# HakimNessah/th_rl

Hardware: NVIDIA B200
Metric: agent-steps/sec (higher is better)
Workload: dtype f32

## Files before the change

th_rl_b200/csrc/thrl.cu:

```cuda
#include <cuda_runtime.h>
#include <stdarg.h>
#include <stdio.h>
#include <string.h>

#include <math.h>
#include <stdlib.h>

#include <algorithm>
#include <array>
#include <cmath>
#include <atomic>
#include <map>
#include <memory>
#include <mutex>
#include <set>
#include <vector>

#include "thrl_device.cuh"
#include "thrl_scan_generic.cuh"
#include "thrl_scan_hbm.cuh"
#include "thrl_scan_lut2.cuh"
#include "thrl_scan_lpc.cuh"
#include "thrl_scan_mixed.cuh"
#include "thrl_scan_pwl.cuh"
// ... 463 lines not shown
    }
    state_of[j] = it->second;
  }
  const int NS = (int)tuples.size();
  if (NS > thrl::kLut2MaxStates) return false;
  std::set<int> rows[2];
  for (auto& t : tuples) { rows[0].insert(t[0]); rows[0].insert(t[1]); rows[1].insert(t[2]); rows[1].insert(t[3]); }
  if (noisy) {
    if (NS + 1 + T > 255) return false;
    for (int a = 0; a < 2; ++a) {
      if (!rows[a].empty() && *rows[a].rbegin() > rmax[a]) return false;
      for (int r = 0; r <= rmax[a]; ++r) rows[a].insert(r);
    }
  }
  std::map<int, int> cidx[2];
  for (int a = 0; a < 2; ++a) {
    if ((int)rows[a].size() > thrl::kLut2MaxRows) return false;
    int c = 0;
    for (int row : rows[a]) {
      if (row < 0 || row > G.agent[a].states) return false;
      p->row_list[a][c] = (uint16_t)row;
      cidx[a][row] = c++;
    }
    p->NR[a] = c;
    const ThrlAgentSpec& s = G.agent[a];
    p->L[a] = s.min_memory > s.capacity ? 0 : (T < s.capacity ? T : s.capacity);
  }
  p->J = J;
  p->NS = NS;
  for (int j = 0; j < J; ++j) p->next_state[j] = (uint8_t)state_of[j];
  for (int s = 0; s < NS; ++s) {
    const auto& t = tuples[s];
    p->state_rows[s] = (uint32_t)cidx[0][t[0]] | ((uint32_t)cidx[0][t[1]] << 8) | ((uint32_t)cidx[1][t[2]] << 16) |
                       ((uint32_t)cidx[1][t[3]] << 24);
  }
  int o = 0;
  p->off_next = o;    o += align_up(2 * J, 16);
  p->off_rowlist = o; o += align_up(2 * (p->NR[0] + p->NR[1]), 16);
  p->off_lutlog = o;  o += J * 32;
  p->off_lutr = o;
  p->cta_bytes_lpc = o + J * 16;
  o += align_up(J * 8, 16);
  p->off_aq = o;      o += align_up((A0 + A1) * 8, 16);
  p->cta_bytes = o;
  o = align_up((p->NR[0] + 2) * A0 * (int)elem, 16);
  p->off_tab1 = o;    o += align_up((p->NR[1] + 2) * A1 * (int)elem, 16);
  p->off_grow = o;    o += align_up(p->NR[0] + p->NR[1] + 4, 16);
  const int nstates = NS + 1 + (noisy ? T : 0);
  p->off_rows = o;    o += align_up(nstates * 4, 16);
  {
    const int gj = align_up((NS + 2) * 4, 16), scr = thrl::kLut2Chunk * 8 + 16;
    p->off_gj = o;    o += gj > scr ? gj : scr;
    p->off_scr = p->off_gj;
  }
  p->off_nt = o;      o += noisy ? align_up(T, 16) : 0;
  p->off_nrec = o;    o += noisy ? align_up(T * 8, 16) : 0;
  p->off_seq = o;     o += noisy ? align_up(T + 1, 16) : 0;
  p->off_rec = o;     o += align_up(2 * T, 16);
  {
    const int pre = align_up(T * 8, 16), olds = align_up(2 * T * (int)elem, 16);
    p->off_old = o;   o += pre > olds ? pre : olds;
  }
  p->warp_bytes = o;
  const int w = (smem_optin - p->cta_bytes) / p->warp_bytes;
  if (w < 2) return false;
  int wmax = elem == 8 ? thrl::Lut2Warps<double>::kMax : thrl::Lut2Warps<float>::kMax;
  if (noisy && wmax > thrl::kLut2NoiseWarps) wmax = thrl::kLut2NoiseWarps;
  *warps = w > wmax ? wmax : w;
  return true;
}

template <typename QT>
int launch_lut2(thrl::Lut2Params& p, int warps, const DeviceInfo& dev, cudaStream_t stream) {
  int grid = dev.sms;
  g_last_wave = (long long)dev.sms * warps;
  const long long needed_ctas = (p.n_runs + warps - 1) / warps;
  if (needed_ctas < grid) {
    warps = (int)((p.n_runs + dev.sms - 1) / dev.sms);
    if (warps < 1) warps = 1;
    grid = (int)((p.n_runs + warps - 1) / warps);
  }
  const size_t smem = (size_t)p.cta_bytes + (size_t)warps * p.warp_bytes;
  const bool small = p.game.agent[0].actions <= 32 && p.game.agent[1].actions <= 32;
  auto kern = p.noisy ? (small ? thrl::qtable_scan_lut2<QT, true, true> : thrl::qtable_scan_lut2<QT, false, true>)
                      : (small ? thrl::qtable_scan_lut2<QT, true> : thrl::qtable_scan_lut2<QT, false>);
  CUDA_TRY(cudaFuncSetAttribute(kern, cudaFuncAttributeMaxDynamicSharedMemorySize, (int)smem));
  g_last_kernel = "lut2";
  kern<<<grid, warps * 32, smem, stream>>>(p);
  CUDA_TRY(cudaGetLastError());
  g_launches.fetch_add(1);
  return THRL_OK;
}

template <typename QT, int GL>
int launch_lpc_gl(thrl::Lut2Params& p, const DeviceInfo& dev, cudaStream_t stream) {
  const ThrlGame& G = p.game;
  const int T = G.max_steps, esz = (int)sizeof(QT);
  thrl::LpcLayout lay;
  lay.cells_max = 0; lay.rows_max = 0;
  int Lmax = 1;
  for (int a = 0; a < 2; ++a) {
    const int cells = (p.NR[a] + 2) * G.agent[a].actions;
    if (cells > lay.cells_max) lay.cells_max = cells;
    if (p.NR[a] + 2 > lay.rows_max) lay.rows_max = p.NR[a] + 2;
    if (p.L[a] > Lmax) Lmax = p.L[a];
  }
  int o = 0;
  lay.off_tab = o;  o += align_up(lay.cells_max * GL * esz, 16);
  lay.off_old = o;  o += align_up(Lmax * GL * esz, 16);
  lay.off_rec = o;  o += align_up(T * GL * 4, 16);
  lay.off_pre = o;  o += align_up(T * GL, 16);
  lay.off_gj = o;   o += align_up((p.NS + 1) * GL * 4, 16);
  lay.off_rows = o; o += align_up((p.NS + 1) * GL * 2, 16);
  lay.off_grow = o; o += align_up(lay.rows_max * GL, 16);
  lay.off_eps = o;  o += align_up(GL * 8, 16);
  lay.off_xrow = o; o += align_up(2 * GL * 2, 16);
  lay.warp_bytes = o;
  int warps = (dev.smem_optin - p.cta_bytes_lpc) / lay.warp_bytes;
  if (warps < 1) return fail(THRL_ERR_UNSUPPORTED, "lpc: one warp group needs %d B of shared memory", lay.warp_bytes);
  if (warps > thrl::kLpcMaxWarps) warps = thrl::kLpcMaxWarps;
  const long long groups = (p.n_runs + GL / 2 - 1) / (GL / 2);
  int grid = dev.sms;
  if ((groups + warps - 1) / warps < grid) {
    warps = (int)((groups + dev.sms - 1) / dev.sms);
    if (warps < 1) warps = 1;
    grid = (int)((groups + warps - 1) / warps);
  }
  const size_t smem = (size_t)p.cta_bytes_lpc + (size_t)warps * lay.warp_bytes;
  const bool a21 = G.agent[0].actions == 21 && G.agent[1].actions == 21;
  auto kern = a21 ? thrl::qtable_scan_lpc<QT, GL, 21> : thrl::qtable_scan_lpc<QT, GL, 0>;
  CUDA_TRY(cudaFuncSetAttribute(kern, cudaFuncAttributeMaxDynamicSharedMemorySize, (int)smem));
  g_last_kernel = "lpc";
  g_last_wave = (long long)grid * warps * (GL / 2);
  kern<<<grid, warps * 32, smem, stream>>>(p, lay);
  CUDA_TRY(cudaGetLastError());
  g_launches.fetch_add(1);
  return THRL_OK;
}
template <typename QT>
int launch_lpc(thrl::Lut2Params& p, const DeviceInfo& dev, cudaStream_t stream) {
  const char* s = getenv("THRL_LPC_GL");
  const int gl = s ? atoi(s) : 8;
  switch (gl) {
    case 4: return launch_lpc_gl<QT, 4>(p, dev, stream);
    case 16: return launch_lpc_gl<QT, 16>(p, dev, stream);
    default: return launch_lpc_gl<QT, 8>(p, dev, stream);
  }
}

template <typename QT>
int launch_mixed(thrl::MixedParams& p, const DeviceInfo& dev, cudaStream_t stream) {
  const ThrlGame& G = p.game;
  const int n = G.n_agents, T = G.max_steps, Hp = p.Hp, esz = (int)sizeof(QT);
  int lut = 0, par = 0, pmax = 0, hmax = 0, amax = 0;
  for (int i = 0; i < n; ++i) {
    const ThrlAgentSpec& s = G.agent[i];
    lut += s.actions;
    p.par_off[i] = 0;
    if (s.kind == THRL_AGENT_QTABLE) continue;
    const int P = s.kind == THRL_AGENT_CAC ? 5 * s.hidden + 3 : 2 * s.hidden + s.actions * s.hidden + s.actions + (s.kind == THRL_AGENT_ACTORCRITIC ? s.hidden + 1 : 0);
    p.par_off[i] = par;
    par += align_up(P, 4);
    if (P > pmax) pmax = P;
    if (s.hidden > hmax) hmax = s.hidden;
    if (s.actions > amax) amax = s.actions;
  }
  p.lut_total = lut;
  p.cta_bytes = align_up(2 * lut * 8, 16);
  int o = 0;
  p.off_P = o;    o += align_up(Hp * 8, 16);
// ... 897 lines not shown
```

th_rl_b200/csrc/thrl_scan_lut2.cuh:

```cuda
#pragma once
#include "thrl_device.cuh"

namespace thrl {

constexpr int kLut2MaxJoint = 1024;
constexpr int kLut2MaxStates = 254;
constexpr int kLut2MaxRows = 253;

struct Lut2Params {
  ThrlGame game;
  long long n_runs, run_id0;
  int epoch_begin, E, rng_mode;
  uint32_t k0, k1;
  void* q;
  uint32_t* counter;
  double* eps;
  double* price;
  const double* hp;
  const double* replay_u;
  const int32_t* replay_ra;
  double* rewards_log;
  double* actions_log;
  long long n_log_runs;
  long long* stats;
  int32_t* trace_actions;
  double* trace_rewards;
  double* trace_prices;
  int J, NS, NR[2], L[2];
  uint8_t next_state[kLut2MaxJoint];
  uint32_t state_rows[kLut2MaxStates];
  uint16_t row_list[2][kLut2MaxRows + 3];
  int cta_bytes, warp_bytes;
  int cta_bytes_lpc;
  int off_next, off_rowlist, off_lutlog, off_lutr, off_aq;
  int off_tab1, off_grow, off_rows, off_gj, off_seq, off_rec, off_scr, off_old;
  int noisy;
  int off_nt, off_nrec;
  const double* replay_new_a;
};

constexpr int kLut2MaxWarps = 24;
template <typename QT> struct Lut2Warps { static constexpr int kMax = kLut2MaxWarps; };
template <> struct Lut2Warps<double> { static constexpr int kMax = 16; };
constexpr int kLut2NoiseWarps = 16;
constexpr int kLut2Chunk = 16;

template <typename QT, bool kSmallA>
__device__ __forceinline__ QT lut2_row_max(const QT* row_lane, int A, int lane, bool in) {
  QT m = in ? row_lane[0] : NegInf<QT>::v();
  if (!kSmallA) {
    for (int k = lane + 32; k < A; k += 32) { const QT v = row_lane[k - lane]; m = v > m ? v : m; }
  }
  return warp_max(m);
}
template <typename QT, bool kSmallA>
__device__ __forceinline__ int lut2_row_argmax(const QT* row, int A, int lane, bool in) {
  if (!kSmallA) return row_argmax(row, A, lane);
  const QT v = in ? row[lane] : NegInf<QT>::v();
  const QT wm = warp_max(v);
  return (int)__reduce_min_sync(kFull, (in && v == wm) ? (unsigned)lane : 0xffffffffu);
}

template <typename QT, bool kSmallA, bool kNoise = false>
__global__ void __launch_bounds__(kNoise ? 32 * kLut2NoiseWarps : 32 * Lut2Warps<QT>::kMax, 1) qtable_scan_lut2(const __grid_constant__ Lut2Params p) {
  extern __shared__ __align__(16) unsigned char smem[];
  const ThrlGame& G = p.game;
  const int lane = threadIdx.x & 31, warps_per_cta = blockDim.x >> 5;
  const int warp = __shfl_sync(kFull, (int)(threadIdx.x >> 5), 0);
  const int T = G.max_steps, E = p.E, J = p.J, NS = p.NS;
  const int A0 = G.agent[0].actions, A1 = G.agent[1].actions;
  const int NR0 = p.NR[0], NR1 = p.NR[1];
  const int rng_mode = p.rng_mode;
  const uint32_t key0 = p.k0, key1 = p.k1;

  uint16_t* nextS = reinterpret_cast<uint16_t*>(smem + p.off_next);
  uint16_t* rowlist = reinterpret_cast<uint16_t*>(smem + p.off_rowlist);
  double* lutP = reinterpret_cast<double*>(smem + p.off_lutr);
  double* lutAq = reinterpret_cast<double*>(smem + p.off_aq);
  double* lutLog = reinterpret_cast<double*>(smem + p.off_lutlog);
  {
    const double ab = __ddiv_rn(G.a, G.b);
    for (int j = threadIdx.x; j < J; j += blockDim.x) {
      const int k0 = j / A1, k1 = j - k0 * A1;
      const double x0 = scale_action(k0, A0, G.agent[0].action_lo, G.agent[0].action_hi);
      const double x1 = scale_action(k1, A1, G.agent[1].action_lo, G.agent[1].action_hi);
      const double aq0 = __dmul_rn(ab, x0), aq1 = __dmul_rn(ab, x1);
      const double Q = __dadd_rn(__dadd_rn(0.0, aq0), aq1);
      const double pn = __dsub_rn(G.a, __dmul_rn(G.b, Q));
      const double price = pn > 0.0 ? pn : (pn != pn ? pn : 0.0);
      const double r0 = __dmul_rn(price, aq0), r1 = __dmul_rn(price, aq1);
      lutP[j] = price;
      lutLog[4 * j + 0] = __ddiv_rn(r0, (double)T);
      lutLog[4 * j + 1] = __ddiv_rn(r1, (double)T);
      lutLog[4 * j + 2] = __ddiv_rn(x0, (double)T);
      lutLog[4 * j + 3] = __ddiv_rn(x1, (double)T);
      nextS[j] = (uint16_t)(4u * p.next_state[j]);
    }
    for (int k = threadIdx.x; k < A0 + A1; k += blockDim.x) {
      const ThrlAgentSpec& sa = G.agent[k < A0 ? 0 : 1];
      lutAq[k] = __dmul_rn(ab, scale_action(k < A0 ? k : k - A0, sa.actions, sa.action_lo, sa.action_hi));
    }
    for (int c = threadIdx.x; c < NR0 + NR1; c += blockDim.x)
      rowlist[c] = c < NR0 ? p.row_list[0][c] : p.row_list[1][c - NR0];
  }
  __syncthreads();

  unsigned char* slot = smem + p.cta_bytes + (size_t)warp * p.warp_bytes;
  QT* tab0 = reinterpret_cast<QT*>(slot);
  QT* tab1 = reinterpret_cast<QT*>(slot + p.off_tab1);
  uint8_t* grow = slot + p.off_grow;
  uint32_t* rowsW = reinterpret_cast<uint32_t*>(slot + p.off_rows);
  unsigned char* GJb = slot + p.off_gj;
  uint32_t* GJ = reinterpret_cast<uint32_t*>(GJb);
  uint16_t* rec = reinterpret_cast<uint16_t*>(slot + p.off_rec);
  uint8_t* seq = slot + p.off_seq;
  uint2* pre = reinterpret_cast<uint2*>(slot + p.off_old);
  unsigned char* chunk = slot + p.off_scr;
  QT* olds = reinterpret_cast<QT*>(slot + p.off_old);
  uint8_t* nT = slot + p.off_nt;
  double* nrec = reinterpret_cast<double*>(slot + p.off_nrec);

  const bool in0 = lane < A0, in1 = lane < A1;
  const bool hi_half = lane >= 16;
  const int L0 = p.L[0], L1 = p.L[1];
  const uint32_t dp_b = (uint32_t)A1 | (1u << 8);
  const uint32_t tab0_off = (uint32_t)(reinterpret_cast<unsigned char*>(tab0) - smem);
  const uint32_t tab1_off = (uint32_t)(reinterpret_cast<unsigned char*>(tab1) - smem);
  const uint32_t tab0_lane_off = tab0_off + (uint32_t)sizeof(QT) * (uint32_t)(kSmallA ? (lane < A0 ? lane : A0 - 1) : lane);
// ... 78 lines not shown
    uint32_t sig4 = 4u * (uint32_t)NS;
    int last_k = -1;
    double noise_price = -1.0;

    for (int e = 0; e < E; ++e) {
      const uint32_t eabs = (uint32_t)(p.epoch_begin + e);
      const long long step0 = (r * E + e) * (long long)T;

      const unsigned long long thr0 = u32_unit_threshold(eps0), thr1 = u32_unit_threshold(eps1);
      for (int t = lane; t < T; t += 32) {
        int f0, f1;
        if (rng_mode == THRL_RNG_PHILOX) {
          uint32_t x[4];
          philox4x32_10(gid, eabs, (uint32_t)t, kStreamAct << 16, key0, key1, x);
          f0 = x[0] < thr0 ? (int)__umulhi(x[1], (uint32_t)A0) : -1;
          f1 = x[2] < thr1 ? (int)__umulhi(x[3], (uint32_t)A1) : -1;
        } else if (rng_mode == THRL_RNG_REPLAY_DRAWS) {
          const double2 u = *reinterpret_cast<const double2*>(p.replay_u + (step0 + t) * 2);
          const int2 v = *reinterpret_cast<const int2*>(p.replay_ra + (step0 + t) * 2);
          f0 = u.x < eps0 ? v.x : -1;
          f1 = u.y < eps1 ? v.y : -1;
        } else {
          const int2 v = *reinterpret_cast<const int2*>(p.replay_ra + (step0 + t) * 2);
          f0 = v.x; f1 = v.y;
        }
        pre[t] = make_uint2((f0 < 0 ? 0xffu : 0u) | (f1 < 0 ? 0xff00u : 0u),
                            (uint32_t)(f0 < 0 ? 0 : f0) | ((uint32_t)(f1 < 0 ? 0 : f1) << 8));
      }
      int nK = 0;
      if (kNoise) {
        for (int t0 = 0; t0 < T; t0 += 32) {
          const int t = t0 + lane;
          bool ev = false;
          double na = G.a;
          if (t < T) {
            if (rng_mode == THRL_RNG_PHILOX) {
              uint32_t x[4];
              philox4x32_10(gid, eabs, (uint32_t)t, kStreamEnv << 16, key0, key1, x);
              if (u53(x[0], x[1]) < G.noise_prob) {
                const double lo = __dmul_rn(G.a, 0.7);
                na = __dadd_rn(lo, __dmul_rn(__dsub_rn(G.a, lo), u53(x[2], x[3])));
                ev = true;
              }
            } else if (p.replay_new_a) {
              na = p.replay_new_a[step0 + t];
              ev = __double_as_longlong(na) != __double_as_longlong(G.a);
            }
          }
          const unsigned m = __ballot_sync(kFull, ev);
          if (ev) {
            const int idx = nK + __popc(m & ((1u << lane) - 1u));
            nT[idx] = (uint8_t)t;
            nrec[idx] = na;
          }
          nK += __popc(m);
        }
      }
      __syncwarp();

      const uint32_t sig4_start = sig4;
      double acc = 0.0;
      {
        const uint32_t base = (uint32_t)__cvta_generic_to_shared(smem);
        const uint32_t pre_a = base + (uint32_t)(reinterpret_cast<unsigned char*>(pre) - smem);
        const uint32_t rec_a = base + (uint32_t)(reinterpret_cast<unsigned char*>(rec) - smem);
        const uint32_t gj_a = base + (uint32_t)(GJb - smem);
        const uint32_t log_a = base + (uint32_t)p.off_lutlog + 8u * (uint32_t)(lane & 3);
        uint32_t next_a = base + (uint32_t)p.off_next;
        asm volatile("" : "+r"(next_a));
        const uint32_t log_lane = lane < 4 ? 1u : 0u;
        double lg = 0.0;
        uint32_t kk = 0;
        auto step = [&](uint32_t fx, uint32_t fy) {
          uint32_t gj, s16;
          asm volatile("ld.shared.u32 %0, [%1];" : "=r"(gj) : "r"(gj_a + sig4));
          kk = (gj & fx) | fy;
          const uint32_t joint = __dp4a(kk, dp_b, 0u);
          asm volatile("{ .reg .pred q; setp.ne.u32 q, %2, 0; @q ld.shared.f64 %0, [%1]; }"
                       : "+d"(lg) : "r"(log_a + 32u * joint), "r"(log_lane));
          acc = __dadd_rn(acc, lg);
          asm volatile("ld.shared.u16 %0, [%1];" : "=r"(s16) : "r"(next_a + 2u * joint));
          sig4 = s16;
        };
        if (!kNoise) {
        uint32_t pa = pre_a, ra = rec_a;
#pragma unroll 2
        for (int n2 = T >> 1; n2 > 0; --n2, pa += 16u, ra += 4u) {
          uint32_t f0x, f0y, f1x, f1y;
          asm volatile("ld.shared.v4.u32 {%0, %1, %2, %3}, [%4];" : "=r"(f0x), "=r"(f0y), "=r"(f1x), "=r"(f1y) : "r"(pa));
          step(f0x, f0y);
          const uint32_t ka = kk;
          step(f1x, f1y);
          asm volatile("st.shared.u32 [%0], %1;" ::"r"(ra), "r"(__byte_perm(ka, kk, 0x5410)) : "memory");
        }
        if (T & 1) {
          uint32_t fx, fy;
          asm volatile("ld.shared.v2.u32 {%0, %1}, [%2];" : "=r"(fx), "=r"(fy) : "r"(pa));
          step(fx, fy);
          asm volatile("st.shared.u16 [%0], %1;" ::"r"(ra), "h"((uint16_t)kk) : "memory");
        }
        } else {
          auto single = [&](int t) {
            uint32_t fx, fy;
            asm volatile("ld.shared.v2.u32 {%0, %1}, [%2];" : "=r"(fx), "=r"(fy) : "r"(pre_a + 8u * (uint32_t)t));
            step(fx, fy);
            asm volatile("st.shared.u16 [%0], %1;" ::"r"(rec_a + 2u * (uint32_t)t), "h"((uint16_t)kk) : "memory");
          };
          const double ab = __ddiv_rn(G.a, G.b), Td = (double)T;
          int t = 0;
          for (int k = 0; k <= nK; ++k) {
            const int tn = k < nK ? (int)nT[k] : T;
            if (t < tn && (t & 1)) { single(t); ++t; }
            for (; t + 1 < tn; t += 2) {
              uint32_t f0x, f0y, f1x, f1y;
              asm volatile("ld.shared.v4.u32 {%0, %1, %2, %3}, [%4];" : "=r"(f0x), "=r"(f0y), "=r"(f1x), "=r"(f1y) : "r"(pre_a + 8u * (uint32_t)t));
              step(f0x, f0y);
              const uint32_t ka = kk;
              step(f1x, f1y);
              asm volatile("st.shared.u32 [%0], %1;" ::"r"(rec_a + 2u * (uint32_t)t), "r"(__byte_perm(ka, kk, 0x5410)) : "memory");
            }
            if (t < tn) { single(t); ++t; }
            if (tn < T) {
              uint32_t fx, fy, gj;
              asm volatile("ld.shared.v2.u32 {%0, %1}, [%2];" : "=r"(fx), "=r"(fy) : "r"(pre_a + 8u * (uint32_t)tn));
              asm volatile("ld.shared.u32 %0, [%1];" : "=r"(gj) : "r"(gj_a + sig4));
              kk = (gj & fx) | fy;
              const int k0 = (int)(kk & 0xff), k1 = (int)(kk >> 8);
              const uint32_t joint = __dp4a(kk, dp_b, 0u);
              const double aq0 = __dmul_rn(ab, scale_action(k0, A0, G.agent[0].action_lo, G.agent[0].action_hi));
              const double aq1 = __dmul_rn(ab, scale_action(k1, A1, G.agent[1].action_lo, G.agent[1].action_hi));
              const double na = nrec[k];
              const double pn = __dsub_rn(na, __dmul_rn(G.b, __dadd_rn(__dadd_rn(0.0, aq0), aq1)));
              const double np = pn > 0.0 ? pn : (pn != pn ? pn : 0.0);
              const double r0 = __dmul_rn(np, aq0), r1 = __dmul_rn(np, aq1);
              if (lane < 2) lg = __ddiv_rn(lane == 0 ? r0 : r1, Td);
              else if (lane < 4) lg = lutLog[4 * joint + lane];
              acc = __dadd_rn(acc, lg);
              const int ta0 = act_row(np, (float)G.agent[0].max_state, (float)G.agent[0].states);
              const int tu0 = upd_row(np, G.agent[0].max_state, (double)G.agent[0].states);
              const int ta1 = act_row(np, (float)G.agent[1].max_state, (float)G.agent[1].states);
              const int tu1 = upd_row(np, G.agent[1].max_state, (double)G.agent[1].states);
              __syncwarp();
              if (lane == 0) {
                nrec[k] = np;
                rowsW[NS + 1 + k] = (uint32_t)ta0 | ((uint32_t)tu0 << 8) | ((uint32_t)ta1 << 16) | ((uint32_t)tu1 << 24);
                GJ[NS + 1] = (uint32_t)grow[ta0] | ((uint32_t)grow[NR0 + 2 + ta1] << 8);
                rec[tn] = (uint16_t)kk;
              }
              __syncwarp();
              sig4 = 4u * (uint32_t)(NS + 1);
              t = tn + 1;
            }
          }
        }
        last_k = (int)kk;
      }
      __syncwarp();
      if (kNoise) {
        for (int t = lane; t <= T; t += 32) {
          uint32_t s4 = sig4_start;
          if (t > 0) { const uint32_t kk = rec[t - 1]; s4 = nextS[__dp4a(kk, dp_b, 0u)]; }
          seq[t] = (uint8_t)(s4 >> 2);
        }
        __syncwarp();
        for (int k = lane; k < nK; k += 32) seq[nT[k] + 1] = (uint8_t)(NS + 1 + k);
        __syncwarp();
      }
// ... 145 lines not shown
            const QT v = row[k];
            if (v > m) { m = v; g = k; }
          }
          return g;
        };
        const unsigned w0a = __reduce_or_sync(kFull, dirty0a), w0b = __reduce_or_sync(kFull, dirty0b);
        const unsigned w1a = __reduce_or_sync(kFull, dirty1a), w1b = __reduce_or_sync(kFull, dirty1b);
        const unsigned below = (1u << lane) - 1u;
        const int n0a = __popc(w0a), n0 = n0a + __popc(w0b), n1a = n0 + __popc(w1a), nd = n1a + __popc(w1b);
        uint8_t* dlist = reinterpret_cast<uint8_t*>(olds);
        if ((w0a >> lane) & 1u) dlist[__popc(w0a & below)] = (uint8_t)lane;
        if ((w0b >> lane) & 1u) dlist[n0a + __popc(w0b & below)] = (uint8_t)(32 + lane);
        if ((w1a >> lane) & 1u) dlist[n0 + __popc(w1a & below)] = (uint8_t)lane;
        if ((w1b >> lane) & 1u) dlist[n1a + __popc(w1b & below)] = (uint8_t)(32 + lane);
        __syncwarp();
        for (int i = lane; i < nd; i += 32) {
          const bool ag = i >= n0;
          const int c = dlist[i], A = ag ? A1 : A0;
          grow[(ag ? NR0 + 2 : 0) + c] = (uint8_t)scan_row((ag ? tab1 : tab0) + c * A, A);
        }
        if (__any_sync(kFull, dirty_all0))
          for (int c = 64 + lane; c < NR0 + 2; c += 32) grow[c] = (uint8_t)scan_row(tab0 + c * A0, A0);
        if (__any_sync(kFull, dirty_all1))
          for (int c = 64 + lane; c < NR1 + 2; c += 32) grow[NR0 + 2 + c] = (uint8_t)scan_row(tab1 + c * A1, A1);
        __syncwarp();
        if (kNoise && sig4 > 4u * (uint32_t)NS) {
          if (lane == 0) rowsW[NS] = rowsW[NS + nK];
          noise_price = nrec[nK - 1];
          sig4 = 4u * (uint32_t)NS;
          __syncwarp();
        } else if (kNoise) {
          noise_price = -1.0;
        }
        for (int s = lane; s <= NS; s += 32) {
          const uint32_t rw = rowsW[s];
          GJ[s] = (uint32_t)grow[rw & 0xff] | ((uint32_t)grow[NR0 + 2 + ((rw >> 16) & 0xff)] << 8);
        }
      }
      {
        const double epsend0 = hparam(0, 2), epsstep0 = hparam(0, 3), epsend1 = hparam(1, 2), epsstep1 = hparam(1, 3);
        eps0 = __dadd_rn(epsend0, __dmul_rn(__dsub_rn(eps0, epsend0), epsstep0));
        eps1 = __dadd_rn(epsend1, __dmul_rn(__dsub_rn(eps1, epsend1), epsstep1));
      }
      if (lane < 4) {
        const int ag = lane & 1;
        if (r < p.n_log_runs) {
          double* dst = lane < 2 ? p.rewards_log : p.actions_log;
          if (dst) dst[(r * E + e) * 2 + ag] = acc;
        }
        if (p.stats) {
          unsigned long long* s4 = reinterpret_cast<unsigned long long*>(p.stats) + ((size_t)e * 2 + ag) * THRL_STATS_K + (lane < 2 ? 0 : 2);
          atomicAdd(s4 + 0, (unsigned long long)fx_round(__dmul_rn(acc, THRL_STATS_SCALE_SUM)));
          atomicAdd(s4 + 1, (unsigned long long)fx_round(__dmul_rn(__dmul_rn(acc, acc), THRL_STATS_SCALE_SQ)));
        }
      }
      __syncwarp();
    }

    for (int c = 0; c < NR0 + 2; ++c) {
      const int row = table_row0(c);
      if (row >= 0) for (int k = lane; k < A0; k += 32) qg0[(size_t)row * G.agent[0].row_stride + k] = tab0[c * A0 + k];
    }
    for (int c = 0; c < NR1 + 2; ++c) {
      const int row = table_row1(c);
      if (row >= 0) for (int k = lane; k < A1; k += 32) qg1[(size_t)row * G.agent[1].row_stride + k] = tab1[c * A1 + k];
    }
    if (lane == 0) {
      p.eps[r * 2] = eps0;
      p.eps[r * 2 + 1] = eps1;
      if (kNoise && noise_price >= 0.0) {
        p.price[r] = noise_price;
      } else if (last_k >= 0) {
        const double ab = __ddiv_rn(G.a, G.b);
        const double aq0 = __dmul_rn(ab, scale_action(last_k & 0xff, A0, G.agent[0].action_lo, G.agent[0].action_hi));
        const double aq1 = __dmul_rn(ab, scale_action(last_k >> 8, A1, G.agent[1].action_lo, G.agent[1].action_hi));
        const double pn = __dsub_rn(G.a, __dmul_rn(G.b, __dadd_rn(__dadd_rn(0.0, aq0), aq1)));
        p.price[r] = pn > 0.0 ? pn : (pn != pn ? pn : 0.0);
      }
    }
    __syncwarp();
  }
}

}
```

Before: 31.16 billion.

## Add paired-run LUT2 kernel processing two runs per warp with half-warp split

```diff
diff --git a/th_rl_b200/csrc/thrl.cu b/th_rl_b200/csrc/thrl.cu
--- a/th_rl_b200/csrc/thrl.cu
+++ b/th_rl_b200/csrc/thrl.cu
@@ -569,10 +569,21 @@
   }
   const size_t smem = (size_t)p.cta_bytes + (size_t)warps * p.warp_bytes;
   const bool small = p.game.agent[0].actions <= 32 && p.game.agent[1].actions <= 32;
+  g_last_kernel = "lut2";
   auto kern = p.noisy ? (small ? thrl::qtable_scan_lut2<QT, true, true> : thrl::qtable_scan_lut2<QT, false, true>)
-                      : (small ? thrl::qtable_scan_lut2<QT, true> : thrl::qtable_scan_lut2<QT, false>);
+                      : thrl::qtable_scan_lut2<QT, false>;
+  if constexpr (std::is_same<QT, float>::value) {
+    if (small && !p.noisy) {
+      CUDA_TRY(cudaFuncSetAttribute(thrl::qtable_scan_lut2_pair, cudaFuncAttributeMaxDynamicSharedMemorySize, (int)smem));
+      thrl::qtable_scan_lut2_pair<<<grid, (warps + 1) / 2 * 32, smem, stream>>>(p, warps);
+      CUDA_TRY(cudaGetLastError());
+      g_launches.fetch_add(1);
+      return THRL_OK;
+    }
+  } else if (small && !p.noisy) {
+    kern = thrl::qtable_scan_lut2<QT, true>;
+  }
   CUDA_TRY(cudaFuncSetAttribute(kern, cudaFuncAttributeMaxDynamicSharedMemorySize, (int)smem));
-  g_last_kernel = "lut2";
   kern<<<grid, warps * 32, smem, stream>>>(p);
   CUDA_TRY(cudaGetLastError());
   g_launches.fetch_add(1);
diff --git a/th_rl_b200/csrc/thrl_scan_lut2.cuh b/th_rl_b200/csrc/thrl_scan_lut2.cuh
--- a/th_rl_b200/csrc/thrl_scan_lut2.cuh
+++ b/th_rl_b200/csrc/thrl_scan_lut2.cuh
@@ -600,4 +600,494 @@
   }
 }
 
+constexpr int kLut2PairWarps = kLut2MaxWarps / 2;
+
+__global__ void __launch_bounds__(32 * kLut2PairWarps, 1) qtable_scan_lut2_pair(const __grid_constant__ Lut2Params p, int slots) {
+  using QT = float;
+  extern __shared__ __align__(16) unsigned char smem[];
+  const ThrlGame& G = p.game;
+  const int lane = threadIdx.x & 31;
+  const int warp = __shfl_sync(kFull, (int)(threadIdx.x >> 5), 0);
+  const int T = G.max_steps, E = p.E, J = p.J, NS = p.NS;
+  const int A0 = G.agent[0].actions, A1 = G.agent[1].actions;
+  const int NR0 = p.NR[0], NR1 = p.NR[1];
+  const int rng_mode = p.rng_mode;
+  const uint32_t key0 = p.k0, key1 = p.k1;
+
+  uint16_t* nextS = reinterpret_cast<uint16_t*>(smem + p.off_next);
+  uint16_t* rowlist = reinterpret_cast<uint16_t*>(smem + p.off_rowlist);
+  double* lutP = reinterpret_cast<double*>(smem + p.off_lutr);
+  double* lutAq = reinterpret_cast<double*>(smem + p.off_aq);
+  double* lutLog = reinterpret_cast<double*>(smem + p.off_lutlog);
+  {
+    const double ab = __ddiv_rn(G.a, G.b);
+    for (int j = threadIdx.x; j < J; j += blockDim.x) {
+      const int k0 = j / A1, k1 = j - k0 * A1;
+      const double x0 = scale_action(k0, A0, G.agent[0].action_lo, G.agent[0].action_hi);
+      const double x1 = scale_action(k1, A1, G.agent[1].action_lo, G.agent[1].action_hi);
+      const double aq0 = __dmul_rn(ab, x0), aq1 = __dmul_rn(ab, x1);
+      const double Q = __dadd_rn(__dadd_rn(0.0, aq0), aq1);
+      const double pn = __dsub_rn(G.a, __dmul_rn(G.b, Q));
+      const double price = pn > 0.0 ? pn : (pn != pn ? pn : 0.0);
+      const double r0 = __dmul_rn(price, aq0), r1 = __dmul_rn(price, aq1);
+      lutP[j] = price;
+      lutLog[4 * j + 0] = __ddiv_rn(r0, (double)T);
+      lutLog[4 * j + 1] = __ddiv_rn(r1, (double)T);
+      lutLog[4 * j + 2] = __ddiv_rn(x0, (double)T);
+      lutLog[4 * j + 3] = __ddiv_rn(x1, (double)T);
+      nextS[j] = (uint16_t)(4u * p.next_state[j]);
+    }
+    for (int k = threadIdx.x; k < A0 + A1; k += blockDim.x) {
+      const ThrlAgentSpec& sa = G.agent[k < A0 ? 0 : 1];
+      lutAq[k] = __dmul_rn(ab, scale_action(k < A0 ? k : k - A0, sa.actions, sa.action_lo, sa.action_hi));
+    }
+    for (int c = threadIdx.x; c < NR0 + NR1; c += blockDim.x)
+      rowlist[c] = c < NR0 ? p.row_list[0][c] : p.row_list[1][c - NR0];
+  }
+  __syncthreads();
+
+  const bool hi_half = lane >= 16;
+  const int li = lane & (kLut2Chunk - 1);
+  const int L0 = p.L[0], L1 = p.L[1];
+  const uint32_t dp_b = (uint32_t)A1 | (1u << 8);
+  const uint32_t col0 = 4u * (uint32_t)(lane < A0 ? lane : A0 - 1), col1 = 4u * (uint32_t)(lane < A1 ? lane : A1 - 1);
+  const uint32_t smem_base = (uint32_t)__cvta_generic_to_shared(smem);
+  auto rec_of = [&](uint32_t so) { return reinterpret_cast<uint16_t*>(smem + so + p.off_rec); };
+  auto rows_of = [&](uint32_t so) { return reinterpret_cast<uint32_t*>(smem + so + p.off_rows); };
+  auto grow_of = [&](uint32_t so) { return smem + so + p.off_grow; };
+  auto gj_of = [&](uint32_t so) { return reinterpret_cast<uint32_t*>(smem + so + p.off_gj); };
+  auto olds_of = [&](uint32_t so) { return reinterpret_cast<QT*>(smem + so + p.off_old); };
+  auto tab_of = [&](uint32_t so, int ag) { return reinterpret_cast<QT*>(smem + so + (ag ? p.off_tab1 : 0)); };
+
+  const long long total_slots = (long long)gridDim.x * slots;
+  for (long long r0 = (long long)blockIdx.x * slots + 2 * warp; r0 < p.n_runs; r0 += total_slots) {
+    const bool live1 = 2 * warp + 1 < slots && r0 + 1 < p.n_runs;
+    const long long r1 = live1 ? r0 + 1 : r0;
+    const uint32_t so0 = (uint32_t)p.cta_bytes + (uint32_t)(2 * warp) * (uint32_t)p.warp_bytes;
+    const uint32_t so1 = live1 ? so0 + (uint32_t)p.warp_bytes : so0;
+    const uint32_t so_me = hi_half ? so1 : so0;
+    const int nr = live1 ? 2 : 1;
+    auto hparam = [&](long long r, int ag, int k) -> double {
+      if (p.hp) return __ldg(p.hp + r * 8 + ag * 4 + k);
+      const ThrlAgentSpec& s = G.agent[ag];
+      return k == 0 ? s.alpha : k == 1 ? s.gamma : k == 2 ? s.eps_end : s.eps_step;
+    };
+    double eps00 = p.eps[r0 * 2], eps01 = p.eps[r0 * 2 + 1], eps10 = p.eps[r1 * 2], eps11 = p.eps[r1 * 2 + 1];
+
+    auto find = [&](const uint16_t* rl, int NRa, int row) -> int {
+      int res = -1;
+      for (int c0 = 0; c0 < NRa; c0 += 32) {
+        const unsigned f = __ballot_sync(kFull, c0 + lane < NRa && rl[c0 + lane] == row);
+        if (f) { res = c0 + __ffs(f) - 1; break; }
+      }
+      return res;
+    };
+    auto init_rows = [&](double price_in, int& x00, int& x01, int& x10, int& x11) -> uint32_t {
+      x00 = x01 = x10 = x11 = -1;
+      const int ta0 = act_row(price_in, (float)G.agent[0].max_state, (float)G.agent[0].states);
+      const int tu0 = upd_row(price_in, G.agent[0].max_state, (double)G.agent[0].states);
+      const int ta1 = act_row(price_in, (float)G.agent[1].max_state, (float)G.agent[1].states);
+      const int tu1 = upd_row(price_in, G.agent[1].max_state, (double)G.agent[1].states);
+      int c0 = find(rowlist, NR0, ta0);
+      if (c0 < 0) { c0 = NR0; x00 = ta0; }
+      int c1 = find(rowlist, NR0, tu0);
+      if (c1 < 0) { if (tu0 == ta0) c1 = c0; else { c1 = NR0 + 1; x01 = tu0; } }
+      int c2 = find(rowlist + NR0, NR1, ta1);
+      if (c2 < 0) { c2 = NR1; x10 = ta1; }
+      int c3 = find(rowlist + NR0, NR1, tu1);
+      if (c3 < 0) { if (tu1 == ta1) c3 = c2; else { c3 = NR1 + 1; x11 = tu1; } }
+      return (uint32_t)c0 | ((uint32_t)c1 << 8) | ((uint32_t)c2 << 16) | ((uint32_t)c3 << 24);
+    };
+    int x000, x001, x010, x011, x100, x101, x110, x111;
+    const uint32_t initw0 = init_rows(p.price[r0], x000, x001, x010, x011);
+    const uint32_t initw1 = init_rows(p.price[r1], x100, x101, x110, x111);
+    auto table_row = [&](bool h, int ag, int c) -> int {
+      if (ag == 0) return c < NR0 ? (int)rowlist[c] : c == NR0 ? (h ? x100 : x000) : (h ? x101 : x001);
+      return c < NR1 ? (int)rowlist[NR0 + c] : c == NR1 ? (h ? x110 : x010) : (h ? x111 : x011);
+    };
+    auto gtab = [&](bool h, int ag) {
+      QT* q = reinterpret_cast<QT*>(p.q) + (h ? r1 : r0) * G.run_stride;
+      return ag ? q + G.agent[1].table_offset : q;
+    };
+
+#pragma unroll
+    for (int h = 0; h < nr; ++h) {
+      const uint32_t so = h ? so1 : so0;
+#pragma unroll
+      for (int ag = 0; ag < 2; ++ag) {
+        const int Aa = ag ? A1 : A0, NRa = ag ? NR1 : NR0;
+        const QT* qg = gtab(h, ag);
+        QT* tab = tab_of(so, ag);
+        for (int c = 0; c < NRa + 2; ++c) {
+          const int row = table_row(h, ag, c);
+          if (row >= 0) for (int k = lane; k < Aa; k += 32) tab[c * Aa + k] = qg[(size_t)row * G.agent[ag].row_stride + k];
+        }
+      }
+      uint32_t* rowsW = rows_of(so);
+      for (int s = lane; s < NS; s += 32) rowsW[s] = p.state_rows[s];
+      if (lane == 0) rowsW[NS] = h ? initw1 : initw0;
+      __syncwarp();
+#pragma unroll
+      for (int ag = 0; ag < 2; ++ag) {
+        const int Aa = ag ? A1 : A0, NRa = ag ? NR1 : NR0;
+        for (int c = 0; c < NRa + 2; ++c) {
+          if (table_row(h, ag, c) >= 0) {
+            const int g = lut2_row_argmax<QT, true>(tab_of(so, ag) + c * Aa, Aa, lane, lane < Aa);
+            if (lane == 0) grow_of(so)[(ag ? NR0 + 2 : 0) + c] = (uint8_t)g;
+          }
+        }
+      }
+      __syncwarp();
+    }
+    auto greedy_pairs = [&]() {
+      for (int i = lane; i < nr * (NS + 1); i += 32) {
+        const bool h = i > NS;
+        const int s = h ? i - NS - 1 : i;
+        const uint32_t so = h ? so1 : so0;
+        const uint32_t rw = rows_of(so)[s];
+        const uint8_t* grow = grow_of(so);
+        gj_of(so)[s] = (uint32_t)grow[rw & 0xff] | ((uint32_t)grow[NR0 + 2 + ((rw >> 16) & 0xff)] << 8);
+      }
+    };
+    greedy_pairs();
+    __syncwarp();
+
+    uint32_t sig4 = 4u * (uint32_t)NS;
+    uint32_t kk = 0;
+
+    for (int e = 0; e < E; ++e) {
+      const uint32_t eabs = (uint32_t)(p.epoch_begin + e);
+      const long long step00 = (r0 * E + e) * (long long)T, step01 = (r1 * E + e) * (long long)T;
+
+      {
+        const unsigned long long t00 = u32_unit_threshold(eps00), t01 = u32_unit_threshold(eps01);
+        const unsigned long long t10 = u32_unit_threshold(eps10), t11 = u32_unit_threshold(eps11);
+        const uint32_t gid0 = (uint32_t)(p.run_id0 + r0), gid1 = (uint32_t)(p.run_id0 + r1);
+        for (int i = lane; i < nr * T; i += 32) {
+          const bool h = i >= T;
+          const int t = h ? i - T : i;
+          const long long st = (h ? step01 : step00) + t;
+          int f0, f1;
+          if (rng_mode == THRL_RNG_PHILOX) {
+            uint32_t x[4];
+            philox4x32_10(h ? gid1 : gid0, eabs, (uint32_t)t, kStreamAct << 16, key0, key1, x);
+            f0 = x[0] < (h ? t10 : t00) ? (int)__umulhi(x[1], (uint32_t)A0) : -1;
+            f1 = x[2] < (h ? t11 : t01) ? (int)__umulhi(x[3], (uint32_t)A1) : -1;
+          } else if (rng_mode == THRL_RNG_REPLAY_DRAWS) {
+            const double2 u = *reinterpret_cast<const double2*>(p.replay_u + st * 2);
+            const int2 v = *reinterpret_cast<const int2*>(p.replay_ra + st * 2);
+            f0 = u.x < (h ? eps10 : eps00) ? v.x : -1;
+            f1 = u.y < (h ? eps11 : eps01) ? v.y : -1;
+          } else {
+            const int2 v = *reinterpret_cast<const int2*>(p.replay_ra + st * 2);
+            f0 = v.x; f1 = v.y;
+          }
+          reinterpret_cast<uint2*>(smem + (h ? so1 : so0) + p.off_old)[t] =
+              make_uint2((f0 < 0 ? 0xffu : 0u) | (f1 < 0 ? 0xff00u : 0u), (uint32_t)(f0 < 0 ? 0 : f0) | ((uint32_t)(f1 < 0 ? 0 : f1) << 8));
+        }
+      }
+      __syncwarp();
+
+      const uint32_t s4s0 = __shfl_sync(kFull, sig4, 0), s4s1 = __shfl_sync(kFull, sig4, 16);
+      double acc = 0.0;
+      {
+        const uint32_t pre_a = smem_base + so_me + (uint32_t)p.off_old;
+        const uint32_t rec_a = smem_base + so_me + (uint32_t)p.off_rec;
+        const uint32_t gj_a = smem_base + so_me + (uint32_t)p.off_gj;
+        const uint32_t log_a = smem_base + (uint32_t)p.off_lutlog + 8u * (uint32_t)(lane & 3);
+        uint32_t next_a = smem_base + (uint32_t)p.off_next;
+        asm volatile("" : "+r"(next_a));
+        const uint32_t log_lane = (lane & 15) < 4 ? 1u : 0u;
+        double lg = 0.0;
+        auto step = [&](uint32_t fx, uint32_t fy) {
+          uint32_t gj, s16;
+          asm volatile("ld.shared.u32 %0, [%1];" : "=r"(gj) : "r"(gj_a + sig4));
+          kk = (gj & fx) | fy;
+          const uint32_t joint = __dp4a(kk, dp_b, 0u);
+          asm volatile("{ .reg .pred q; setp.ne.u32 q, %2, 0; @q ld.shared.f64 %0, [%1]; }"
+                       : "+d"(lg) : "r"(log_a + 32u * joint), "r"(log_lane));
+          acc = __dadd_rn(acc, lg);
+          asm volatile("ld.shared.u16 %0, [%1];" : "=r"(s16) : "r"(next_a + 2u * joint));
+          sig4 = s16;
+        };
+        uint32_t pa = pre_a, ra = rec_a;
+#pragma unroll 2
+        for (int n2 = T >> 1; n2 > 0; --n2, pa += 16u, ra += 4u) {
+          uint32_t f0x, f0y, f1x, f1y;
+          asm volatile("ld.shared.v4.u32 {%0, %1, %2, %3}, [%4];" : "=r"(f0x), "=r"(f0y), "=r"(f1x), "=r"(f1y) : "r"(pa));
+          step(f0x, f0y);
+          const uint32_t ka = kk;
+          step(f1x, f1y);
+          asm volatile("st.shared.u32 [%0], %1;" ::"r"(ra), "r"(__byte_perm(ka, kk, 0x5410)) : "memory");
+        }
+        if (T & 1) {
+          uint32_t fx, fy;
+          asm volatile("ld.shared.v2.u32 {%0, %1}, [%2];" : "=r"(fx), "=r"(fy) : "r"(pa));
+          step(fx, fy);
+          asm volatile("st.shared.u16 [%0], %1;" ::"r"(ra), "h"((uint16_t)kk) : "memory");
+        }
+      }
+      __syncwarp();
+      auto rows_before = [&](uint32_t so, uint32_t s4start, int j) -> uint32_t {
+        const uint32_t led = nextS[__dp4a((uint32_t)rec_of(so)[j > 0 ? j - 1 : 0], dp_b, 0u)];
+        return *reinterpret_cast<const uint32_t*>(smem + so + p.off_rows + (j > 0 ? led : s4start));
+      };
+
+      if (p.trace_actions || p.trace_rewards || p.trace_prices) {
+        const double ab = __ddiv_rn(G.a, G.b);
+        for (int i = lane; i < nr * T; i += 32) {
+          const bool h = i >= T;
+          const int t = h ? i - T : i;
+          const long long st = (h ? step01 : step00) + t;
+          const uint16_t kt = rec_of(h ? so1 : so0)[t];
+          const int k0 = kt & 0xff, k1 = kt >> 8, joint = k0 * A1 + k1;
+          if (p.trace_actions) { p.trace_actions[st * 2] = k0; p.trace_actions[st * 2 + 1] = k1; }
+          if (p.trace_rewards) {
+            p.trace_rewards[st * 2] = __dmul_rn(lutP[joint], lutAq[k0]);
+            p.trace_rewards[st * 2 + 1] = __dmul_rn(lutP[joint], lutAq[A0 + k1]);
+          }
+          if (p.trace_prices) {
+            const double aq0 = __dmul_rn(ab, scale_action(k0, A0, G.agent[0].action_lo, G.agent[0].action_hi));
+            const double aq1 = __dmul_rn(ab, scale_action(k1, A1, G.agent[1].action_lo, G.agent[1].action_hi));
+            const double pn = __dsub_rn(G.a, __dmul_rn(G.b, __dadd_rn(__dadd_rn(0.0, aq0), aq1)));
+            p.trace_prices[st] = pn > 0.0 ? pn : (pn != pn ? pn : 0.0);
+          }
+        }
+      }
+
+      unsigned long long d00 = 0, d01 = 0, d10 = 0, d11 = 0;
+      bool all00 = false, all01 = false, all10 = false, all11 = false;
+      const bool pass_rows = L0 == L1;
+      if (!pass_rows)
+        for (int i = lane; i < nr * L1; i += 32) {
+          const bool h = i >= L1;
+          const int jj = h ? i - L1 : i;
+          const uint32_t so = h ? so1 : so0;
+          reinterpret_cast<uint32_t*>(olds_of(so) + 2 * jj + 1)[0] = rows_before(so, h ? s4s1 : s4s0, T - L1 + jj);
+        }
+      for (int i = lane; i < nr * L0; i += 32) {
+        const bool h = i >= L0;
+        const int jj = h ? i - L0 : i, j = T - L0 + jj;
+        const uint32_t so = h ? so1 : so0;
+        const uint32_t rw = rows_before(so, h ? s4s1 : s4s0, j);
+        const int k = rec_of(so)[j] & 0xff, cu = (rw >> 8) & 0xff;
+        QT* olds = olds_of(so);
+        olds[2 * jj] = tab_of(so, 0)[cu * A0 + k];
+        if (pass_rows) reinterpret_cast<uint32_t*>(olds + 2 * jj + 1)[0] = rw;
+        if (p.counter)
+          atomicAdd(p.counter + (h ? r1 : r0) * G.run_stride + (size_t)table_row(h, 0, cu) * G.agent[0].row_stride + k, 1u);
+        const unsigned long long bit = cu < 64 ? 1ull << cu : 0ull;
+        if (h) { d01 |= bit; all01 |= cu >= 64; } else { d00 |= bit; all00 |= cu >= 64; }
+      }
+      for (int i = lane; i < nr * L1; i += 32) {
+        const bool h = i >= L1;
+        const int jj = h ? i - L1 : i, j = T - L1 + jj;
+        const uint32_t so = h ? so1 : so0;
+        QT* olds = olds_of(so);
+        const int k = rec_of(so)[j] >> 8, cu = reinterpret_cast<const uint32_t*>(olds + 2 * jj + 1)[0] >> 24;
+        olds[2 * jj + 1] = tab_of(so, 1)[cu * A1 + k];
+        if (p.counter)
+          atomicAdd(p.counter + (h ? r1 : r0) * G.run_stride + G.agent[1].table_offset + (size_t)table_row(h, 1, cu) * G.agent[1].row_stride + k, 1u);
+        const unsigned long long bit = cu < 64 ? 1ull << cu : 0ull;
+        if (h) { d11 |= bit; all11 |= cu >= 64; } else { d10 |= bit; all10 |= cu >= 64; }
+      }
+      __syncwarp();
+
+      auto expand = [&](uint32_t so, int jj, int ag, int La, double oma, uint32_t& rw_carry, uint32_t& row_off,
+                        uint32_t& cell_addr, double2& v) {
+        const int j = T - La + jj;
+        const uint32_t kk = rec_of(so)[j];
+        const uint32_t rn = *reinterpret_cast<const uint32_t*>(smem + so + p.off_rows + nextS[__dp4a(kk, dp_b, 0u)]);
+        const uint32_t below = __shfl_up_sync(kFull, rn, 1, kLut2Chunk);
+        const uint32_t rw = li ? below : rw_carry;
+        rw_carry = __shfl_sync(kFull, rn, kLut2Chunk - 1);
+        const int joint = (int)__dp4a(kk, dp_b, 0u);
+        const uint32_t sel_row = ag ? 0x4443u : 0x4441u;
+        const int Aa = ag ? A1 : A0, k = (int)__byte_perm(kk, 0u, ag ? 0x4441u : 0x4440u);
+        const int cu = (int)__byte_perm(rw, 0u, sel_row), cn = (int)__byte_perm(rn, 0u, sel_row);
+        row_off = (uint32_t)(cn * Aa) * (uint32_t)sizeof(QT);
+        cell_addr = so + (uint32_t)(ag ? p.off_tab1 : 0) + (uint32_t)(cu * Aa + k) * (uint32_t)sizeof(QT);
+        const double rew = __dmul_rn(lutP[joint], lutAq[ag ? A0 + k : k]);
+        v = make_double2(rew, __dmul_rn(oma, (double)olds_of(so)[2 * jj + ag]));
+        asm volatile("" : "+d"(v.x), "+d"(v.y), "+r"(cell_addr));
+      };
+      auto row_max = [&](uint32_t lane_off, uint32_t row_off) -> QT {
+        return warp_max(*reinterpret_cast<const QT*>(smem + (lane_off + row_off)));
+      };
+
+      if (L0 == L1) {
+        const int ag = hi_half;
+        double al0 = hparam(r0, ag, 0), ga0 = hparam(r0, ag, 1), om0 = __dsub_rn(1.0, al0);
+        double al1 = hparam(r1, ag, 0), ga1 = hparam(r1, ag, 1), om1 = __dsub_rn(1.0, al1);
+        asm volatile("" : "+d"(al0), "+d"(ga0), "+d"(om0), "+d"(al1), "+d"(ga1), "+d"(om1));
+        const uint32_t lt00 = so0 + col0, lt01 = so0 + (uint32_t)p.off_tab1 + col1;
+        const uint32_t lt10 = so1 + col0, lt11 = so1 + (uint32_t)p.off_tab1 + col1;
+        uint32_t carry0 = rows_before(so0, s4s0, T - L0), carry1 = rows_before(so1, s4s1, T - L0);
+        for (int c0 = 0; c0 < L0; c0 += kLut2Chunk) {
+          const int n = L0 - c0 < kLut2Chunk ? L0 - c0 : kLut2Chunk;
+          uint32_t ro0, ce0, ro1, ce1;
+          double2 v0, v1;
+          expand(so0, min(c0 + li, L0 - 1), ag, L0, om0, carry0, ro0, ce0, v0);
+          expand(so1, min(c0 + li, L0 - 1), ag, L0, om1, carry1, ro1, ce1, v1);
+          const uint32_t oth0 = __shfl_xor_sync(kFull, ro0, 16), oth1 = __shfl_xor_sync(kFull, ro1, 16);
+          if (lane < n) {
+            *reinterpret_cast<uint2*>(smem + so0 + p.off_scr + lane * 8) = make_uint2(ro0, oth0);
+            *reinterpret_cast<uint2*>(smem + so1 + p.off_scr + lane * 8) = make_uint2(ro1, oth1);
+          }
+          __syncwarp();
+          uint32_t cp0 = smem_base + so0 + (uint32_t)p.off_scr, cp1 = smem_base + so1 + (uint32_t)p.off_scr;
+          int cd = li;
+          uint32_t nx0, ny0, nx1, ny1;
+          asm volatile("ld.shared.v2.u32 {%0, %1}, [%2];" : "=r"(nx0), "=r"(ny0) : "r"(cp0));
+          asm volatile("ld.shared.v2.u32 {%0, %1}, [%2];" : "=r"(nx1), "=r"(ny1) : "r"(cp1));
+#pragma unroll 2
+          for (int j = n; j > 0; --j, --cd) {
+            const uint32_t ox0 = nx0, oy0 = ny0, ox1 = nx1, oy1 = ny1;
+            cp0 += 8u;
+            cp1 += 8u;
+            asm volatile("ld.shared.v2.u32 {%0, %1}, [%2];" : "=r"(nx0), "=r"(ny0) : "r"(cp0));
+            asm volatile("ld.shared.v2.u32 {%0, %1}, [%2];" : "=r"(nx1), "=r"(ny1) : "r"(cp1));
+            const QT m00 = row_max(lt00, ox0), m01 = row_max(lt01, oy0);
+            const QT m10 = row_max(lt10, ox1), m11 = row_max(lt11, oy1);
+            const double mx0 = (double)(hi_half ? m01 : m00), mx1 = (double)(hi_half ? m11 : m10);
+            const double nv0 = __dadd_rn(v0.y, __dmul_rn(al0, __dadd_rn(v0.x, __dmul_rn(ga0, mx0))));
+            const double nv1 = __dadd_rn(v1.y, __dmul_rn(al1, __dadd_rn(v1.x, __dmul_rn(ga1, mx1))));
+            if (cd == 0) {
+              *reinterpret_cast<QT*>(smem + ce0) = (QT)nv0;
+              *reinterpret_cast<QT*>(smem + ce1) = (QT)nv1;
+            }
+            __syncwarp();
+          }
+        }
+      } else {
+        for (int ag = 0; ag < 2; ++ag) {
+          const int La = ag ? L1 : L0;
+          const double al0 = hparam(r0, ag, 0), ga0 = hparam(r0, ag, 1), om0 = __dsub_rn(1.0, al0);
+          const double al1 = hparam(r1, ag, 0), ga1 = hparam(r1, ag, 1), om1 = __dsub_rn(1.0, al1);
+          const uint32_t lt0 = so0 + (ag ? (uint32_t)p.off_tab1 + col1 : col0), lt1 = so1 + (ag ? (uint32_t)p.off_tab1 + col1 : col0);
+          uint32_t carry0 = La == 0 ? 0u : rows_before(so0, s4s0, T - La), carry1 = La == 0 ? 0u : rows_before(so1, s4s1, T - La);
+          for (int c0 = 0; c0 < La; c0 += kLut2Chunk) {
+            const int n = La - c0 < kLut2Chunk ? La - c0 : kLut2Chunk;
+            uint32_t ro0, ce0, ro1, ce1;
+            double2 v0, v1;
+            expand(so0, min(c0 + li, La - 1), ag, La, om0, carry0, ro0, ce0, v0);
+            expand(so1, min(c0 + li, La - 1), ag, La, om1, carry1, ro1, ce1, v1);
+            if (lane < n) {
+              *reinterpret_cast<uint32_t*>(smem + so0 + p.off_scr + lane * 8) = ro0;
+              *reinterpret_cast<uint32_t*>(smem + so1 + p.off_scr + lane * 8) = ro1;
+            }
+            __syncwarp();
+            for (int j = 0; j < n; ++j) {
+              const double mx0 = (double)row_max(lt0, *reinterpret_cast<const uint32_t*>(smem + so0 + p.off_scr + j * 8));
+              const double mx1 = (double)row_max(lt1, *reinterpret_cast<const uint32_t*>(smem + so1 + p.off_scr + j * 8));
+              const double nv0 = __dadd_rn(v0.y, __dmul_rn(al0, __dadd_rn(v0.x, __dmul_rn(ga0, mx0))));
+              const double nv1 = __dadd_rn(v1.y, __dmul_rn(al1, __dadd_rn(v1.x, __dmul_rn(ga1, mx1))));
+              if (lane == j) {
+                *reinterpret_cast<QT*>(smem + ce0) = (QT)nv0;
+                *reinterpret_cast<QT*>(smem + ce1) = (QT)nv1;
+              }
+              __syncwarp();
+            }
+          }
+        }
+      }
+
+      {
+        auto scan_row = [&](const QT* row, int A) -> int {
+          QT m = row[0];
+          int g = 0;
+#pragma unroll 4
+          for (int k = 1; k < A; ++k) {
+            const QT v = row[k];
+            if (v > m) { m = v; g = k; }
+          }
+          return g;
+        };
+        const unsigned below = (1u << lane) - 1u;
+        auto list = [&](uint32_t so, unsigned long long d0, unsigned long long d1, int& n0) -> int {
+          const unsigned w0a = __reduce_or_sync(kFull, (unsigned)d0), w0b = __reduce_or_sync(kFull, (unsigned)(d0 >> 32));
+          const unsigned w1a = __reduce_or_sync(kFull, (unsigned)d1), w1b = __reduce_or_sync(kFull, (unsigned)(d1 >> 32));
+          const int n0a = __popc(w0a), n1a = n0a + __popc(w0b) + __popc(w1a);
+          n0 = n0a + __popc(w0b);
+          uint8_t* dlist = reinterpret_cast<uint8_t*>(olds_of(so));
+          if ((w0a >> lane) & 1u) dlist[__popc(w0a & below)] = (uint8_t)lane;
+          if ((w0b >> lane) & 1u) dlist[n0a + __popc(w0b & below)] = (uint8_t)(32 + lane);
+          if ((w1a >> lane) & 1u) dlist[n0 + __popc(w1a & below)] = (uint8_t)lane;
+          if ((w1b >> lane) & 1u) dlist[n1a + __popc(w1b & below)] = (uint8_t)(32 + lane);
+          return n1a + __popc(w1b);
+        };
+        int n00, n01 = 0;
+        const int nd0 = list(so0, d00, d10, n00);
+        const int nd1 = live1 ? list(so1, d01, d11, n01) : 0;
+        __syncwarp();
+        for (int i = lane; i < nd0 + nd1; i += 32) {
+          const bool h = i >= nd0;
+          const int ii = h ? i - nd0 : i;
+          const uint32_t so = h ? so1 : so0;
+          const bool ag = ii >= (h ? n01 : n00);
+          const int c = reinterpret_cast<const uint8_t*>(olds_of(so))[ii], A = ag ? A1 : A0;
+          grow_of(so)[(ag ? NR0 + 2 : 0) + c] = (uint8_t)scan_row(tab_of(so, ag) + c * A, A);
+        }
+#pragma unroll
+        for (int h = 0; h < 2; ++h) {
+          const uint32_t so = h ? so1 : so0;
+          if (__any_sync(kFull, h ? all01 : all00))
+            for (int c = 64 + lane; c < NR0 + 2; c += 32) grow_of(so)[c] = (uint8_t)scan_row(tab_of(so, 0) + c * A0, A0);
+          if (__any_sync(kFull, h ? all11 : all10))
+            for (int c = 64 + lane; c < NR1 + 2; c += 32) grow_of(so)[NR0 + 2 + c] = (uint8_t)scan_row(tab_of(so, 1) + c * A1, A1);
+        }
+        __syncwarp();
+        greedy_pairs();
+      }
+      eps00 = __dadd_rn(hparam(r0, 0, 2), __dmul_rn(__dsub_rn(eps00, hparam(r0, 0, 2)), hparam(r0, 0, 3)));
+      eps01 = __dadd_rn(hparam(r0, 1, 2), __dmul_rn(__dsub_rn(eps01, hparam(r0, 1, 2)), hparam(r0, 1, 3)));
+      eps10 = __dadd_rn(hparam(r1, 0, 2), __dmul_rn(__dsub_rn(eps10, hparam(r1, 0, 2)), hparam(r1, 0, 3)));
+      eps11 = __dadd_rn(hparam(r1, 1, 2), __dmul_rn(__dsub_rn(eps11, hparam(r1, 1, 2)), hparam(r1, 1, 3)));
+      if ((lane & 15) < 4 && (!hi_half || live1)) {
+        const int ag = lane & 1;
+        const bool rw_lane = (lane & 15) < 2;
+        const long long r = hi_half ? r1 : r0;
+        if (r < p.n_log_runs) {
+          double* dst = rw_lane ? p.rewards_log : p.actions_log;
+          if (dst) dst[(r * E + e) * 2 + ag] = acc;
+        }
+        if (p.stats) {
+          unsigned long long* s4 = reinterpret_cast<unsigned long long*>(p.stats) + ((size_t)e * 2 + ag) * THRL_STATS_K + (rw_lane ? 0 : 2);
+          atomicAdd(s4 + 0, (unsigned long long)fx_round(__dmul_rn(acc, THRL_STATS_SCALE_SUM)));
+          atomicAdd(s4 + 1, (unsigned long long)fx_round(__dmul_rn(__dmul_rn(acc, acc), THRL_STATS_SCALE_SQ)));
+        }
+      }
+      __syncwarp();
+    }
+
+#pragma unroll
+    for (int h = 0; h < nr; ++h) {
+      const uint32_t so = h ? so1 : so0;
+#pragma unroll
+      for (int ag = 0; ag < 2; ++ag) {
+        const int Aa = ag ? A1 : A0, NRa = ag ? NR1 : NR0;
+        QT* qg = gtab(h, ag);
+        const QT* tab = tab_of(so, ag);
+        for (int c = 0; c < NRa + 2; ++c) {
+          const int row = table_row(h, ag, c);
+          if (row >= 0) for (int k = lane; k < Aa; k += 32) qg[(size_t)row * G.agent[ag].row_stride + k] = tab[c * Aa + k];
+        }
+      }
+    }
+    if (lane == 0 || (lane == 16 && live1)) {
+      const long long r = hi_half ? r1 : r0;
+      p.eps[r * 2] = hi_half ? eps10 : eps00;
+      p.eps[r * 2 + 1] = hi_half ? eps11 : eps01;
+      if (E > 0) {
+        const double ab = __ddiv_rn(G.a, G.b);
+        const double aq0 = __dmul_rn(ab, scale_action(kk & 0xff, A0, G.agent[0].action_lo, G.agent[0].action_hi));
+        const double aq1 = __dmul_rn(ab, scale_action(kk >> 8, A1, G.agent[1].action_lo, G.agent[1].action_hi));
+        const double pn = __dsub_rn(G.a, __dmul_rn(G.b, __dadd_rn(__dadd_rn(0.0, aq0), aq1)));
+        p.price[r] = pn > 0.0 ? pn : (pn != pn ? pn : 0.0);
+      }
+    }
+    __syncwarp();
+  }
 }
+
+}
```

Result: slower. 30.10 billion, median of 6 (-3.4%).

## Parallelize sequential LUT scan across warp lanes using pointer-jumping successor tables

Applied to the files above, without the earlier changes.

```diff
diff --git a/th_rl_b200/csrc/thrl_scan_lut2.cuh b/th_rl_b200/csrc/thrl_scan_lut2.cuh
--- a/th_rl_b200/csrc/thrl_scan_lut2.cuh
+++ b/th_rl_b200/csrc/thrl_scan_lut2.cuh
@@ -44,6 +44,7 @@
 template <> struct Lut2Warps<double> { static constexpr int kMax = 16; };
 constexpr int kLut2NoiseWarps = 16;
 constexpr int kLut2Chunk = 16;
+constexpr int kLut2MaxEvents = 12;
 
 template <typename QT, bool kSmallA>
 __device__ __forceinline__ QT lut2_row_max(const QT* row_lane, int A, int lane, bool in) {
@@ -288,7 +289,100 @@
           asm volatile("ld.shared.u16 %0, [%1];" : "=r"(s16) : "r"(next_a + 2u * joint));
           sig4 = s16;
         };
-        if (!kNoise) {
+        unsigned evm0 = 0, evm1 = 0, evm2 = 0, evm3 = 0;
+        bool par = false;
+        if (!kNoise && T > 0 && T <= 128 && NS < 64) {
+          const uint32_t* prew = reinterpret_cast<const uint32_t*>(pre);
+          auto evmask = [&](int t0) { const int t = t0 + lane; return __ballot_sync(kFull, t < T && prew[2 * t] != 0xffffu); };
+          evm0 = evmask(0); evm1 = evmask(32); evm2 = evmask(64); evm3 = evmask(96);
+          par = __popc(evm0) + __popc(evm1) + __popc(evm2) + __popc(evm3) <= kLut2MaxEvents;
+        }
+        if (!kNoise && par) {
+          uint32_t fp[5];
+          {
+            auto succ = [&](uint32_t s) -> uint32_t {
+              uint32_t n4 = 4u * s;
+              if (s <= (uint32_t)NS) {
+                uint32_t gj;
+                asm volatile("ld.shared.u32 %0, [%1];" : "=r"(gj) : "r"(gj_a + 4u * s));
+                asm volatile("ld.shared.u16 %0, [%1];" : "=r"(n4) : "r"(next_a + 2u * __dp4a(gj, dp_b, 0u)));
+              }
+              return n4 >> 2;
+            };
+            fp[0] = succ((uint32_t)lane) | (succ((uint32_t)lane + 32u) << 8);
+          }
+          auto fwd = [&](uint32_t v, uint32_t s) -> uint32_t {
+            uint32_t r;
+            asm("prmt.b32 %0, %1, 0, %2;" : "=r"(r) : "r"(__shfl_sync(kFull, v, (int)s)), "r"((s >> 5) + 0x4440u));
+            return r;
+          };
+#pragma unroll
+          for (int k = 1; k < 5; ++k) fp[k] = fwd(fp[k - 1], fp[k - 1] & 0xffu) | (fwd(fp[k - 1], fp[k - 1] >> 8) << 8);
+          auto lift = [&](uint32_t s, uint32_t d) -> uint32_t {
+#pragma unroll
+            for (int k = 0; k < 5; ++k) {
+              const uint32_t n = fwd(fp[k], s);
+              s = (d >> k) & 1u ? n : s;
+            }
+            return s;
+          };
+
+          uint32_t sc = sig4_start >> 2;
+          unsigned m = evm0;
+          for (int c0 = 0; c0 < T; c0 += 32) {
+            const int t = c0 + lane;
+            uint32_t fx = 0xffffu, fy = 0u;
+            if (t < T) asm volatile("ld.shared.v2.u32 {%0, %1}, [%2];" : "=r"(fx), "=r"(fy) : "r"(pre_a + 8u * (uint32_t)t));
+            uint32_t st = lift(sc, (uint32_t)lane), kt, n4;
+            auto play = [&]() {
+              uint32_t gj;
+              asm volatile("ld.shared.u32 %0, [%1];" : "=r"(gj) : "r"(gj_a + 4u * st));
+              kt = (gj & fx) | fy;
+              asm volatile("ld.shared.u16 %0, [%1];" : "=r"(n4) : "r"(next_a + 2u * __dp4a(kt, dp_b, 0u)));
+            };
+            play();
+            for (unsigned mw = m; mw != 0u; mw &= mw - 1u) {
+              const int i = __ffs(mw) - 1;
+              const uint32_t nx = lift(__shfl_sync(kFull, n4, i) >> 2, (uint32_t)(lane - i - 1));
+              st = lane > i ? nx : st;
+              play();
+            }
+            if (t < T) asm volatile("st.shared.u16 [%0], %1;" ::"r"(rec_a + 2u * (uint32_t)t), "h"((uint16_t)kt) : "memory");
+            sc = __shfl_sync(kFull, n4, 31) >> 2;
+            m = c0 == 0 ? evm1 : c0 == 32 ? evm2 : evm3;
+          }
+          __syncwarp();
+          {
+            const uint32_t lq = log_a, wq = (32u * (uint32_t)A1) | (32u << 16);
+            auto add = [&](uint32_t a) {
+              asm volatile("ld.shared.f64 %0, [%1];" : "=d"(lg) : "r"(a));
+              acc = __dadd_rn(acc, lg);
+            };
+            auto eight = [&](int t) {
+              uint32_t r0, r1, r2, r3;
+              asm volatile("ld.shared.v4.u32 {%0, %1, %2, %3}, [%4];" : "=r"(r0), "=r"(r1), "=r"(r2), "=r"(r3) : "r"(rec_a + 2u * (uint32_t)t));
+              add(__dp2a_lo(wq, r0, lq)); add(__dp2a_hi(wq, r0, lq));
+              add(__dp2a_lo(wq, r1, lq)); add(__dp2a_hi(wq, r1, lq));
+              add(__dp2a_lo(wq, r2, lq)); add(__dp2a_hi(wq, r2, lq));
+              add(__dp2a_lo(wq, r3, lq)); add(__dp2a_hi(wq, r3, lq));
+            };
+            int t = 0;
+#pragma unroll 1
+            for (; t + 32 <= T; t += 32) { eight(t); eight(t + 8); eight(t + 16); eight(t + 24); }
+#pragma unroll 1
+            for (; t + 8 <= T; t += 8) eight(t);
+#pragma unroll 1
+            for (; t < T; ++t) {
+              uint32_t r0;
+              asm volatile("ld.shared.u16 %0, [%1];" : "=r"(r0) : "r"(rec_a + 2u * (uint32_t)t));
+              add(__dp2a_lo(wq, r0, lq));
+            }
+          }
+          uint32_t s16;
+          asm volatile("ld.shared.u16 %0, [%1];" : "=r"(kk) : "r"(rec_a + 2u * (uint32_t)(T - 1)));
+          asm volatile("ld.shared.u16 %0, [%1];" : "=r"(s16) : "r"(next_a + 2u * __dp4a(kk, dp_b, 0u)));
+          sig4 = s16;
+        } else if (!kNoise) {
         uint32_t pa = pre_a, ra = rec_a;
 #pragma unroll 2
         for (int n2 = T >> 1; n2 > 0; --n2, pa += 16u, ra += 4u) {
```

Result: faster. 31.16 billion before, 34.24 billion after, median of 6 (+9.9%).
